# esq4/nind-denoise

Hardware: AMD Instinct MI355X
Metric: megapixels/sec denoised, UtNet cs=256 on 24 MP frames, 1/2/4/8 MI355X (higher is better)
Workload: dtype f32; 1 GPU; configs[1]: one 6000x4000 (24.0 MP) fp32 frame per step, f32 storage in the conv stack (fp32 accumulate), UtNet(funit=64,PReLU) random-init (seed 123), cs=264 (nearest valid to the named size; the reference rejects 256 / 512) ucs=200 ol=64 -> 1276 tiles/frame, tiles per conv-stack launch 256, crop->infer->stitch device resident (frame and canvas in HBM); every tile's input is the whole cs x cs cro; tiles_per_frame=1276, parallelism=single GPU

## Files before the change

nind_denoise_amd/csrc/aux_kernels.hip:

```cpp
#include "nd_common.h"

typedef float f32x4 __attribute__((ext_vector_type(4)));
typedef __bf16 bf16x8 __attribute__((ext_vector_type(8)));
typedef _Float16 f16x8 __attribute__((ext_vector_type(8)));

template <int DT> struct Elem { typedef f32x4 vec; static constexpr int N = 4; typedef float scalar; };
template <> struct Elem<ND_BF16> { typedef bf16x8 vec; static constexpr int N = 8; typedef __bf16 scalar; };
template <> struct Elem<ND_F16> { typedef f16x8 vec; static constexpr int N = 8; typedef _Float16 scalar; };
#define ND_DISPATCH_DT(dt, CALL)                     \
    switch (dt) {                                    \
        case ND_F32: { constexpr int DT = ND_F32; CALL; break; }   \
        case ND_BF16: { constexpr int DT = ND_BF16; CALL; break; } \
        case ND_F16: { constexpr int DT = ND_F16; CALL; break; }   \
        default: ND_FAIL(ND_EINVAL, "unsupported storage type %d", dt); \
    }

static int make_geo(int W, int H, int cs, int ucs, int ol, TileGeo *g) {
    if (W <= 0 || H <= 0 || cs <= 0 || ucs <= 0 || ol < 0) ND_FAIL(ND_EINVAL, "tile grid: non-positive size");
    if (ucs - ol <= 0) ND_FAIL(ND_EINVAL, "tile grid: ucs (%d) must exceed the overlap (%d)", ucs, ol);
    if (cs < ucs) ND_FAIL(ND_EINVAL, "tile grid: cs (%d) < ucs (%d)", cs, ucs);
    g->W = W; g->H = H; g->cs = cs; g->ucs = ucs; g->ol = ol;
    g->stride = ucs - ol;
    g->pad = (cs - ucs) / 2;
    g->cols = ceil_div_py(W - ucs, g->stride) + 1;
// ... 166 lines not shown

int nd_launch_gather_edges(const float *img, int W, int H, int cs, int ucs, int ol, int set, int first, int count, const QpBuf &dst,
                           hipStream_t s) {
    TileGeo g;
    ND_TRY(make_geo(W, H, cs, ucs, ol, &g));
    const bool corners = set == ND_EDGE_CORNERS;
    bool ok = img && dst.base && dst.dt == ND_F32 && dst.pad == 0 && dst.Hb >= 1 && dst.Wb >= 1 && dst.used() <= dst.pstride &&
              dst.B <= 65535 && dst.Hb <= 65535 && first >= 0 && count > 0 && cs >= 3;
    if (set == ND_EDGE_ROWS) ok = ok && first + count <= g.rows && dst.B == 2 * count && dst.Hb <= cs + 4;
    else if (set == ND_EDGE_COLS) ok = ok && first + count <= g.rows && dst.B == 2 * g.cols && dst.Wb <= cs + 4;
    else ok = ok && corners && first + count <= g.cols * g.rows && dst.B == 4 * count && dst.Hb <= cs + 4 && dst.Wb <= cs + 4;
    if (!ok) ND_FAIL(ND_EINVAL, "gather_edges: bad set %d, range [%d,+%d) or destination", set, first, count);
    dim3 grid((dst.Wb + 255) / 256, dst.Hb, dst.B);
    hipLaunchKernelGGL(k_gather_edges, grid, dim3(256), 0, s, img, g, set, first, (f32x4 *)dst.base, dst.Hb, dst.Wb);
    ND_HIP(hipGetLastError());
    return ND_OK;
}

struct SpliceArgs {
    const f32x4 *src;
    f32x4 *dst;
    long src_np, dst_np;
    int src_Hb, src_Wb, src_pad, dst_Hb, dst_Wb, dst_pad;
    int tile_begin, cols, row0, r0, c0, rows, ccols, planes, dst_img0;
    SpliceMap m;
    int band_rows;
    long slot_elems;
};
__global__ void k_splice(SpliceArgs a) {
    const int k = blockIdx.x * blockDim.x + threadIdx.x;
    if (k >= a.rows * a.ccols) return;
    const int r = a.r0 + k / a.ccols, c = a.c0 + k % a.ccols;
    const int t = blockIdx.y / a.planes, p = blockIdx.y - t * a.planes;
    const int i = a.tile_begin + t;
    const int yi = i / a.cols, xi = i - yi * a.cols;
    const int band = a.band_rows > 0 ? yi / a.band_rows : 0, yrel = yi - (a.band_rows > 0 ? band * a.band_rows : a.row0);
    const int simg = a.m.img_t * t + a.m.img_y * yrel + a.m.img_x * xi + a.m.img_add;
    const int sy = yrel * a.m.step_y + r + a.m.oy + a.src_pad, sx = xi * a.m.step_x + c + a.m.ox + a.src_pad;
    const long si = (long)p * a.src_np + (band & 1) * a.slot_elems + ((long)simg * a.src_Hb + sy) * a.src_Wb + sx;
    a.dst[(long)p * a.dst_np + ((long)(a.dst_img0 + t) * a.dst_Hb + r + a.dst_pad) * a.dst_Wb + c + a.dst_pad] = a.src[si];
}

int nd_launch_splice(const QpBuf &src, int src_p0, const QpBuf &dst, int dst_p0, int planes, int tile_begin, int tile_count, int cols,
                     int row0, const SpliceMap &m, int r0, int r1, int c0, int c1, hipStream_t s, int band_rows, long slot_elems,
                     int dst_img0) {
    const int sH = src.Hb - 2 * src.pad, sW = src.Wb - 2 * src.pad, dH = dst.Hb - 2 * dst.pad, dW = dst.Wb - 2 * dst.pad;
    bool ok = src.dt == ND_F32 && dst.dt == ND_F32 && tile_begin >= 0 && cols > 0 && tile_count > 0 && dst_img0 >= 0 &&
              dst_img0 + tile_count <= dst.B && dst.used() <= dst.np() && src.used() <= src.np() && planes > 0 &&
              src_p0 >= 0 && src_p0 + planes <= src.planes && dst_p0 >= 0 && dst_p0 + planes <= dst.planes &&
              r0 >= 0 && c0 >= 0 && r1 > r0 && c1 > c0 && r1 <= dH && c1 <= dW && band_rows >= 0 &&
              (band_rows == 0 || slot_elems >= 0) && (long)tile_count * planes <= 65535;
    for (int t = 0; t < tile_count && ok; ++t) {
        const int yi = (tile_begin + t) / cols, xi = (tile_begin + t) % cols;
        const int yrel = yi - (band_rows > 0 ? yi / band_rows * band_rows : row0);
        const int simg = m.img_t * t + m.img_y * yrel + m.img_x * xi + m.img_add, y = yrel * m.step_y + m.oy, x = xi * m.step_x + m.ox;
        if (band_rows > 0 && (yi / band_rows & 1)) ok = slot_elems >= src.used() && slot_elems + src.used() <= src.np();
        ok = ok && yrel >= 0 && simg >= 0 && simg < src.B && y + r0 >= 0 && y + r1 - 1 < sH && x + c0 >= 0 && x + c1 - 1 < sW;
    }
    if (!ok) ND_FAIL(ND_EINVAL, "splice: region [%d,%d) x [%d,%d) of %d tiles x %d planes outside its source / destination", r0, r1, c0, c1,
                     tile_count, planes);
    SpliceArgs a;
    a.src = (const f32x4 *)src.base + (long)src_p0 * src.np();
    a.dst = (f32x4 *)dst.base + (long)dst_p0 * dst.np();
    a.src_np = src.np(); a.dst_np = dst.np();
    a.src_Hb = src.Hb; a.src_Wb = src.Wb; a.src_pad = src.pad;
    a.dst_Hb = dst.Hb; a.dst_Wb = dst.Wb; a.dst_pad = dst.pad;
    a.tile_begin = tile_begin; a.cols = cols; a.row0 = row0; a.m = m; a.dst_img0 = dst_img0;
    a.r0 = r0; a.c0 = c0; a.rows = r1 - r0; a.ccols = c1 - c0; a.planes = planes;
    a.band_rows = band_rows; a.slot_elems = slot_elems;
    dim3 grid(((r1 - r0) * (c1 - c0) + 255) / 256, tile_count * planes);
    hipLaunchKernelGGL(k_splice, grid, dim3(256), 0, s, a);
    ND_HIP(hipGetLastError());
    return ND_OK;
}

__host__ __device__ static inline long skip_origin(int i, int cols, int band_rows, int step, int Wb, int dpad, long slot_elems) {
    const int yi = i / cols, xi = i - yi * cols, band = yi / band_rows;
    return (band & 1) * slot_elems + (long)((yi - band * band_rows) * step + dpad) * Wb + xi * step + dpad;
}
__global__ void k_skip_origins(int tile_begin, int tile_count, int cols, int band_rows, int step, int Wb, int dpad, long slot_elems,
                               int *__restrict__ table) {
    const int t = blockIdx.x * blockDim.x + threadIdx.x;
    if (t >= tile_count) return;
    table[t] = (int)skip_origin(tile_begin + t, cols, band_rows, step, Wb, dpad, slot_elems);
}

int nd_launch_skip_origins(const QpBuf &src, int dst_pad, int tile_begin, int tile_count, int cols, int band_rows, int step, long slot_elems,
                           int *table, long *origin_max, hipStream_t s) {
    const int dpad = src.pad - dst_pad;
    if (!table || tile_begin < 0 || tile_count <= 0 || cols <= 0 || band_rows <= 0 || step < 0 || dpad < 0 || slot_elems < 0 || src.B != 1)
        ND_FAIL(ND_EINVAL, "skip_origins: bad tile range [%d,+%d) / %d rows per band", tile_begin, tile_count, band_rows);
    long omax = 0;
    for (int t = 0; t < tile_count; ++t) {
        const long o = skip_origin(tile_begin + t, cols, band_rows, step, src.Wb, dpad, slot_elems);
        omax = o > omax ? o : omax;
    }
// ... 499 lines not shown
```

nind_denoise_amd/csrc/conv_w2d.hip:

```cpp
#include "conv_qp.inc"

namespace {

typedef float f32x2 __attribute__((ext_vector_type(2)));

constexpr int kR = 8;
constexpr int kS = 16;
constexpr int kRI = kR + 2;
constexpr int kVPlane = kRI * kS * 16;
constexpr int kVPos = 2 * kVPlane;
constexpr int kVBytes = 6 * kVPos;
constexpr int kTaps = 18;
constexpr int kMTB = 2;
constexpr int kWBytes = kMTB * kTaps * 1024;
constexpr int kStage = kWBytes + kVBytes;
constexpr int kStages = 2;
constexpr int kScratch = 2048;
constexpr int kLds = kStages * kStage + 8 * kScratch;
constexpr int kDmaAt = 4;
constexpr int kXfAt = 12;
constexpr int kSlots = 4 * 32 * 4;

template <int OFF> __device__ __forceinline__ void glds16o(const void *g, void *l) {
    __builtin_amdgcn_global_load_lds((const __attribute__((address_space(1))) void *)g, (__attribute__((address_space(3))) void *)l, 16, OFF, 0);
// ... 6 lines not shown
    v[0] = 4.f * d[0] - 5.f * d[2] + d[4];
    v[1] = s34 - 4.f * s12;
    v[2] = d43 + 4.f * d12;
    v[3] = d42 + 2.f * d31;
    v[4] = d42 - 2.f * d31;
    v[5] = 4.f * d[1] - 5.f * d[3] + d[5];
}
__device__ __forceinline__ void w4_out(const float *m, float *y) {
    const float a = m[1] + m[2], b = m[1] - m[2], c = m[3] + m[4], e = m[3] - m[4];
    y[0] = m[0] + a + c;
    y[1] = b + 2.f * e;
    y[2] = a + 4.f * c;
    y[3] = b + 8.f * e + m[5];
}

__device__ __forceinline__ unsigned long long stamp() {
    unsigned long long t;
    __builtin_amdgcn_sched_barrier(0);
    asm volatile("s_memtime %0\n\ts_waitcnt lgkmcnt(0)" : "=s"(t)::"memory");
    __builtin_amdgcn_sched_barrier(0);
    return t;
}

struct Strip { int img, y0, x0; bool ok; };

template <int DBG, bool SRC2 = false, bool ADD = false>
__global__ __launch_bounds__(512) void conv_w2d(ConvParams p) {
    extern __shared__ __attribute__((aligned(16))) char smem[];
    const int lane = threadIdx.x & 63;
    const int wave = __builtin_amdgcn_readfirstlane(threadIdx.x >> 6);
    const int wm = wave >> 2, wn = wave & 3;
    const int j = lane & 31, h = lane >> 5;
    const int nwg = gridDim.x;
    const int bid = blockIdx.x;
    const int vb = (nwg % 8 == 0) ? (bid % 8) * (nwg / 8) + bid / 8 : bid;

    const int nchunks = p.KB;
    const int nitems = p.nitems;
    const int my_items = vb < nitems ? (nitems - vb + nwg - 1) / nwg : 0;
    struct Item { int tile, c0, c1, slice; };
    auto decode = [&](int w) -> Item {
        Item it;
        if (w < p.split_first) {
            it.tile = w; it.c0 = 0; it.c1 = nchunks; it.slice = -1;
        } else {
            const int u = w - p.split_first;
// ... 465 lines not shown
    const int Hfull = d.in.Hb - 2, Wfull = d.in.Wb - 2;
    if (Hfull < 1 || Wfull < 1) ND_FAIL(ND_EINVAL, "w2d: input smaller than the kernel");
    ND_TRY(nd_check_roi("w2d", d, Hfull, Wfull, d.pool != nullptr, "a pooled layer"));
    const bool roi = d.roi_rows > 0;
    const int Hv = roi ? d.roi_rows : Hfull, Wpx = roi ? d.roi_cols : Wfull, Wg = (Wpx + 3) / 4, NB = (Hv + kR - 1) / kR;
    if (d.pre && (roi || d.pool)) ND_FAIL(ND_EINVAL, "w2d: a pre-activation copy goes with whole, unpooled layers only");
    if (d.cout % 4) ND_FAIL(ND_EINVAL, "w2d: cout must be a multiple of 4");
    ND_TRY(nd_check_in_planes("w2d", d, KB, true, true));
    const bool src2 = d.in2.base != nullptr, add = d.add.base != nullptr;
    if (add && (d.pool || d.pre || src2))
        ND_FAIL(ND_EINVAL, "w2d: a layer with an addend source is neither pooled nor keeps a pre-activation copy nor has a second input source");
    if (add) ND_TRY(nd_check_add("w2d", d, (long)(d.roi_r0 + Hv - 1 + d.add.pad) * d.add.Wb + d.roi_c0 + Wpx - 1 + d.add.pad + 1));
    if (src2 && (d.pool || d.pre)) ND_FAIL(ND_EINVAL, "w2d: a layer with a second input source is neither pooled nor keeps a pre-activation copy");
    if (src2) ND_TRY(nd_check_in2("w2d", d, KB, (long)(d.roi_r0 + (NB - 1) * kR + kRI - 1) * d.in2.Wb + d.roi_c0 + 4 * (Wg - 1) + 6));
    ND_TRY(nd_check_out("w2d", d, Hfull, Wfull, false));
    ND_TRY(nd_check_int32("w2d", d.in));
    if (2 * d.in.np() * 16 + 65536 >= (1L << 32)) ND_FAIL(ND_EINVAL, "w2d: input too large for 32-bit byte offsets");

    int dev = 0, ncus = 0;
    ND_TRY(nd_device(&dev, &ncus));
    void (*fn)(ConvParams) = add ? conv_w2d<0, false, true> : src2 ? conv_w2d<0, true> : conv_w2d<0>;
#ifdef ND_QP_STAMPS
    static const int dbg_all = getenv("ND_W2D_DBG") ? atoi(getenv("ND_W2D_DBG")) : 0;
    const int dbg_env = src2 || add ? 0 : dbg_all;
    switch (dbg_env) {
        case 1: fn = conv_w2d<1>; break;
        case 2: fn = conv_w2d<2>; break;
        case 4: fn = conv_w2d<4>; break;
        case 8: fn = conv_w2d<8>; break;
        case 16: fn = conv_w2d<16>; break;
        case 24: fn = conv_w2d<24>; break;
        case 28: fn = conv_w2d<28>; break;
        case 30: fn = conv_w2d<30>; break;
        case 32: fn = conv_w2d<32>; break;
        case 62: fn = conv_w2d<62>; break;
        case 128: fn = conv_w2d<128>; break;
        case 256: fn = conv_w2d<256>; break;
        default: break;
    }
#endif
    ND_TRY(nd_raise_lds(dev, (const void *)fn, kLds));

    ConvParams p = nd_conv_params(d, KB, d.cout);
    if (roi) {
        p.in += (long)d.roi_r0 * d.in.Wb + d.roi_c0;
        p.out += (long)d.roi_r0 * d.out.Wb + d.roi_c0;
    }
    if (src2) {
        p.in2 = (const f32x4 *)d.in2.base + (long)d.in2_plane0 * d.in2.np() + (roi ? (long)d.roi_r0 * d.in2.Wb + d.roi_c0 : 0);
        p.in2_plane = d.in2.np();
        p.origin2 = d.in2_origin;
        p.kb2 = d.in2_from / 2;
        p.Wb2 = d.in2.Wb;
    }
    if (d.w_kb) {
        p.KBw = d.w_kb;
        p.wpk += (size_t)d.w_kb0 * kTaps * 256;
    }
    if (add) {
        p.add = (const f32x4 *)d.add.base + (long)d.add_plane0 * d.add.np() + (long)((roi ? d.roi_r0 : 0) + d.add.pad) * d.add.Wb +
                (roi ? d.roi_c0 : 0) + d.add.pad;
        p.add_plane = d.add.np();
        p.origin_add = d.add_origin;
        p.W_add = d.add.Wb;
    }
    p.Hv = Hv;
    p.Wv = Wg;
    p.PV = NB * Wg;
    p.wpx = Wpx;
    if (d.pool) {
        ND_TRY(nd_conv_pool("w2d", d, Hv, Wpx, p));
        if (d.pool->used() * 16 >= (1L << 32)) ND_FAIL(ND_EINVAL, "w2d: pooled destination too large for 32-bit byte offsets");
    }
    nd_conv_tiles(p, true, kS, kMTB * 32);
    nd_conv_fastdivs(p);
    const long ntiles = p.tiles_per_problem;
    const long cap = d.part && !d.nosplit && !d.pool && !d.pre ? (long)(d.part_bytes / ((size_t)kMTB * 32 * kSlots * 4)) : 0;
    const long grid = nd_conv_schedule(p, ntiles, KB, ncus, cap);
    p.part = (f32x4 *)d.part;
#ifdef ND_QP_STAMPS
    if (dbg_env == 128) {
        static int printed = 0;
        static const char *const names[6] = {"issue loads + DMA", "MFMA loop", "wait vmcnt", "transform+publish (inside the loop)", "epilogue", "barrier"};
        return nd_stamped_launch(fn, 512, kLds, p, ntiles, KB, ncus, stream, printed++ < 2, nullptr, "[w2d stamps] wave", names, 6, {0, 1, 4});
    }
#endif
    hipLaunchKernelGGL(fn, dim3((unsigned)grid), dim3(512), kLds, stream, p);
    if (p.split_first < ntiles) hipLaunchKernelGGL(k_w2d_split_finish, dim3((unsigned)(ntiles - p.split_first), kMTB * 8), dim3(256), 0, stream, p);
    ND_HIP(hipGetLastError());
    return ND_OK;
}

bool nd_f43_w2d(const QpBuf &in, int cout, bool pre, int flags) {
    return !(flags & ND_FLAG_W1D_REGS) && nd_w2d_ok(in) && (!pre || nd_w2d_tiles(in, cout) >= 512);
}
int nd_launch_conv_f43(const ConvDesc &d, int flags, hipStream_t stream) {
    return nd_f43_w2d(d.in, d.cout, d.pre != nullptr, flags) ? nd_launch_conv_w2d(d, stream) : nd_launch_conv_w1d(4, d, stream);
}
```

nind_denoise_amd/csrc/nd_common.h:

```cpp
#pragma once
#include <hip/hip_runtime.h>

#include <stdarg.h>
#include <stdint.h>
#include <stdio.h>

#include "nind_hip.h"

void nd_set_error(const char *fmt, ...);
#define ND_FAIL(code, ...)        \
    do {                          \
        nd_set_error(__VA_ARGS__); \
        return (code);            \
    } while (0)
#define ND_HIP(call)                                                                         \
    do {                                                                                     \
        hipError_t e_ = (call);                                                              \
        if (e_ != hipSuccess) ND_FAIL(ND_EHIP, "%s failed: %s", #call, hipGetErrorString(e_)); \
    } while (0)
#define ND_TRY(call)        \
    do {                    \
        int r_ = (call);    \
        if (r_ != 0) return r_; \
    } while (0)
// ... 167 lines not shown
int nd_launch_qp_to_nchw(const QpBuf &src, int plane0, float *y, int C, hipStream_t s);
int nd_launch_reflect_pack(const float *x_nchw, int B, int H, int W, const QpBuf &dst, hipStream_t s);
int nd_launch_maxpool2(const QpBuf &src, int src_plane0, int planes, const QpBuf &dst, hipStream_t s);
int nd_launch_final1x1(const QpBuf &src, int cin, const float *w, const float *bias, int crop, float *y_nchw, int H,
                       int W, hipStream_t s, int sigmoid = 0);
int nd_launch_final1x1_stitch(const QpBuf &src, int cin, const float *w, const float *bias, int crop, float *canvas,
                              int width, int height, int cs, int ucs, int ol, int tile_begin, int tile_count,
                              hipStream_t s, int sigmoid = 0, const float *noise_img = nullptr);
int nd_launch_gather_pack(const float *img, int width, int height, int cs, int ucs, int ol, int tile_begin,
                          int tile_count, const QpBuf &dst, hipStream_t s, int border = 2, bool reflect = true);
int nd_launch_gather_band(const float *img, int width, int height, int cs, int ucs, int ol, int band_row0, const QpBuf &dst,
                          hipStream_t s);
enum nd_edge_set { ND_EDGE_ROWS = 0, ND_EDGE_COLS = 1, ND_EDGE_CORNERS = 2 };
int nd_launch_gather_edges(const float *img, int width, int height, int cs, int ucs, int ol, int set, int first, int count,
                           const QpBuf &dst, hipStream_t s);
int nd_launch_skip_origins(const QpBuf &src, int dst_pad, int tile_begin, int tile_count, int cols, int band_rows, int step, long slot_elems,
                           int *table, long *origin_max, hipStream_t s);
struct SpliceMap {
    int step_y = 0, step_x = 0, img_t = 0, img_y = 0, img_x = 0, img_add = 0, oy = 0, ox = 0;
};
int nd_launch_splice(const QpBuf &src, int src_p0, const QpBuf &dst, int dst_p0, int planes, int tile_begin, int tile_count, int cols,
                     int row0, const SpliceMap &m, int r0, int r1, int c0, int c1, hipStream_t s, int band_rows = 0,
                     long slot_elems = 0, int dst_img0 = 0);

int nd_launch_repitch(const QpBuf &src, int src_plane0, int planes, int ss, int sy, int sx, const QpBuf &dst, int oy, int ox, int h, int w,
                      hipStream_t s);
size_t nd_wgrad_partial_floats(int taps, int M, int N, long K, int *ksplit_out, int *cps_out);
int nd_launch_wgrad(const QpBuf &A, int a_plane0, int M, const QpBuf &Bq, int b_plane0, int N, int taps, int taps_total, int tap0,
                    float *partial, size_t partial_floats, float *dw, hipStream_t s);
int nd_launch_channel_sum(const QpBuf &src, int plane0, int C, float *out, float *scratch, hipStream_t s);
int nd_launch_maxpool_bwd_add(const QpBuf &gpool, const QpBuf &fwd, int fwd_plane0, const QpBuf &gfine, int g_plane0, int planes,
                              hipStream_t s);
int nd_launch_final_wgrad(const float *gy, int H, int W, const QpBuf &act, int cin, int crop, float *red, float *dw, float *db,
                          hipStream_t s);
int nd_launch_final_bwd_data(const float *gy, int H, int W, const float *w, int cin, int crop, const QpBuf &g, hipStream_t s);

int nd_launch_bn_train_fwd(const QpBuf &z, const QpBuf &a, int plane0, int cout, float momentum, const float *gamma, const float *beta,
                           float *rm, float *rv, float *stat, float *red, long red_floats, hipStream_t s);
int nd_launch_bn_train_bwd(const QpBuf &g, const QpBuf &a, int plane0, const QpBuf &z, int cout, const float *gamma, const float *stat,
                           float *coef, float *dgamma, float *dbeta, float *red, long red_floats, hipStream_t s);
```

nind_denoise_amd/csrc/utnet_frame.hip:

```cpp
#include <string.h>

#include "nd_common.h"

#include "utnet_net.h"

namespace {

constexpr int kSharedSteps = 6, kLevel2End = 9;
constexpr int kStrip = 16, kStrip2 = 6;
constexpr double kBandBytes = 8.0 * (1 << 30);

struct Level {
    int begin, end;
    Buf in, out;
    int strip;
    int out_shift;
    bool three_pass;
    bool by_side;
};
const Level kLevels[2] = {{0, kSharedSteps, X0, P2, kStrip, 2, false, false}, {kSharedSteps, kLevel2End, P2, P3, kStrip2, 3, true, true}};
struct SkipSpec { Buf cat; int level, edge; };
const SkipSpec kSkips[3] = {{CAT4, 0, 2}, {CAT3, 0, 1}, {CAT2, 1, 1}};
inline int skip_step(Buf cat) {
    for (int i = 0; i < kNumSteps; ++i)
// ... 252 lines not shown
    struct Skip { int step; bool in_place, fold; Form form; } skips[3];
    int skip_planes(int k) const { return pl.buf[kSkips[k].cat].planes / 2; }
    int tile_rows(int b) const { return fp.rows - b * fp.R < fp.R ? fp.rows - b * fp.R : fp.R; }
};

inline Plan level_scratch(const Frame &c, int l, Plan p) {
    p.split = c.pl.split;
    p.wino = c.ws.scratch[l];
    p.wino_bytes = c.fp.lb[l].scratch;
    return p;
}
inline int run_level(const Frame &c, int l, const Plan &p) {
    StackOpts o;
    o.flags = c.flags;
    o.step_begin = kLevels[l].begin;
    o.step_end = kLevels[l].end;
    return run_stack(c.f, c.act, c.dt, c.blob, p, c.s, o);
}
inline void line_image(const Level &lv, int side, int count, int *step, int *add) {
    *step = lv.by_side ? 1 : 2;
    *add = lv.by_side ? side * count : side;
}

int splice_line_inputs(const Frame &c, int l, int nrows, const Plan &band, const Plan &re, const Plan &ce, const Plan &rows, const Plan &cols) {
    const Level &lv = kLevels[l], &up = kLevels[l - 1];
    const Buf in = lv.in;
    const int n = c.tile[in], planes = band.buf[in].planes, h = band.buf[in].Hb, w = band.buf[in].Wb;
    for (int side = 0; side < 2; ++side) {
        const int at = side * (lv.strip - 1), in0 = 1 - side, in1 = lv.strip - side;
        SpliceMap br, lr, bc, lc;
        br.step_y = bc.step_x = c.fp.S >> up.out_shift;
        br.oy = bc.ox = side * (n - lv.strip);
        line_image(up, side, nrows, &lr.img_y, &lr.img_add);
        line_image(up, side, c.fp.cols, &lc.img_x, &lc.img_add);
        lr.oy = lc.ox = -at;
        ND_TRY(nd_launch_splice(band.buf[in], 0, rows.buf[in], 0, planes, 0, nrows, 1, 0, br, in0, in1, 0, w, c.s, 0, 0, side * nrows));
        ND_TRY(nd_launch_splice(re.buf[in], 0, rows.buf[in], 0, planes, 0, nrows, 1, 0, lr, at, at + 1, 0, w, c.s, 0, 0, side * nrows));
        ND_TRY(nd_launch_splice(band.buf[in], 0, cols.buf[in], 0, planes, 0, c.fp.cols, c.fp.cols, 0, bc, 0, h, in0, in1, c.s, 0, 0, side * c.fp.cols));
        ND_TRY(nd_launch_splice(ce.buf[in], 0, cols.buf[in], 0, planes, 0, c.fp.cols, c.fp.cols, 0, lc, 0, h, at, at + 1, c.s, 0, 0, side * c.fp.cols));
    }
    return ND_OK;
}

int build_band(const Frame &c, int b) {
    const FramePlan &fp = c.fp;
    const int row0 = b * fp.R, nrows = c.tile_rows(b), slot = b & 1;
    Plan band, re, ce;
    for (int l = 0; l < c.nlev; ++l) {
        const Level &lv = kLevels[l];
        Plan bp = level_scratch(c, l, band_plan(fp, l, c.f, c.dt, nrows, c.cs, c.ws.band[l], slot));
        if (l == 0)
            ND_TRY(nd_launch_gather_band(c.img, c.W, c.H, c.cs, c.ucs, c.ol, row0, bp.buf[lv.in], c.s));
        else
            bp.buf[lv.in] = band.buf[lv.in];
        ND_TRY(run_level(c, l, bp));
        for (int k = 0; k < 3; ++k)
            if (kSkips[k].level == l && c.skips[k].fold)
                ND_TRY(launch_skip_fold(c.f, c.flags, c.blob, c.bl, c.skips[k].step, c.skips[k].form, bp.buf[kSkips[k].cat], c.skip_planes(k),
                                        c.rois[c.skips[k].step], fp.S >> k, nrows, fp.cols, c.pl.split, c.ws.fold_scratch, fp.fold_bytes, c.s));
        const Plan rows = level_scratch(c, l, row_plan(fp, l, c.f, c.dt, nrows, c.ws.rows[l], slot));
        const Plan cols = level_scratch(c, l, col_plan(fp, l, c.f, c.dt, nrows, c.cs, c.ws.cols[l], slot));
        if (l == 0) {
            ND_TRY(nd_launch_gather_edges(c.img, c.W, c.H, c.cs, c.ucs, c.ol, ND_EDGE_ROWS, row0, nrows, rows.buf[lv.in], c.s));
            ND_TRY(nd_launch_gather_edges(c.img, c.W, c.H, c.cs, c.ucs, c.ol, ND_EDGE_COLS, row0, nrows, cols.buf[lv.in], c.s));
        } else {
            ND_TRY(splice_line_inputs(c, l, nrows, band, re, ce, rows, cols));
        }
        ND_TRY(run_level(c, l, rows));
        ND_TRY(run_level(c, l, cols));
        band = bp;
        re = rows;
        ce = cols;
    }
    return ND_OK;
}

int corner_patches(const Frame &c, int l, const Plan &tp, int t0, int cnt, Plan *cp) {
    const Level &lv = kLevels[l];
    *cp = level_scratch(c, l, corner_plan(l, c.f, c.dt, cnt, c.batch, c.ws.corners[l]));
    if (l == 0) ND_TRY(nd_launch_gather_edges(c.img, c.W, c.H, c.cs, c.ucs, c.ol, ND_EDGE_CORNERS, t0, cnt, cp->buf[lv.in], c.s));
    for (int k = 0; l > 0 && k < 4; ++k) {
        SpliceMap m;
        m.img_t = 1;
        m.oy = (k >> 1) * (c.tile[lv.in] - lv.strip);
        m.ox = (k & 1) * (c.tile[lv.in] - lv.strip);
        ND_TRY(nd_launch_splice(tp.buf[lv.in], 0, cp->buf[lv.in], 0, tp.buf[lv.in].planes, 0, cnt, cnt, 0, m, 0, lv.strip, 0, lv.strip, c.s, 0, 0, k * cnt));
    }
    return run_level(c, l, *cp);
}

int bind_skips(const Frame &c, const Plan &tp, int t0, int cnt, StepSrc2 *src2, int *nsrc2) {
    const FramePlan &fp = c.fp;
    *nsrc2 = 0;
    for (int k = 0; k < 3; ++k) {
        if (kSkips[k].level >= c.nlev) continue;
        const Buf cat = kSkips[k].cat;
        const QpBuf &src = c.full[kSkips[k].level].buf[cat];
        const int planes = c.skip_planes(k), tstep = fp.S >> k, *win = fp.win[k];
        if (!c.skips[k].in_place && !c.skips[k].fold) {
            SpliceMap m;
            m.step_y = m.step_x = tstep;
            ND_TRY(nd_launch_splice(src, planes, tp.buf[cat], planes, planes, t0, cnt, fp.cols, 0, m, win[0], win[1], win[0], win[1], c.s, fp.R,
                                    slot_elems(src, fp.slots)));
            continue;
        }
        StepSrc2 &q = src2[(*nsrc2)++];
        q.step = c.skips[k].step;
        q.buf = src;
        q.plane0 = q.from = planes;
        q.addend = c.skips[k].fold;
        if (q.addend) {
            q.plane0 = 0;
            q.buf.pad = 1;
        }
        q.origin = c.ws.origins[k];
        ND_TRY(nd_launch_skip_origins(src, tp.buf[cat].pad, t0, cnt, fp.cols, fp.R, tstep, slot_elems(src, fp.slots), c.ws.origins[k],
                                      &q.origin_max, c.s));
    }
    return ND_OK;
}

int assemble_output(const Frame &c, int l, const Plan &tp, const Plan &cp, int t0, int cnt) {
    const FramePlan &fp = c.fp;
    const Level &lv = kLevels[l];
    const QpBuf &dst = tp.buf[lv.out], &bt = c.full[l].buf[lv.out];
    const int n = c.tile[lv.out], step = fp.S >> lv.out_shift, per_band = fp.R * fp.cols;
    SpliceMap whole;
    whole.step_y = whole.step_x = step;
    ND_TRY(nd_launch_splice(bt, 0, dst, 0, dst.planes, t0, cnt, fp.cols, 0, whole, 0, n, 0, n, c.s, fp.R, slot_elems(bt, fp.slots)));
    for (int b = t0 / per_band; b <= (t0 + cnt - 1) / per_band; ++b) {
        const int lo = t0 > b * per_band ? t0 : b * per_band, hi = t0 + cnt < (b + 1) * per_band ? t0 + cnt : (b + 1) * per_band;
        const int row0 = b * fp.R, nrows = c.tile_rows(b);
        const QpBuf rl = row_plan(fp, l, c.f, c.dt, nrows, c.ws.rows[l], b & 1).buf[lv.out];
        const QpBuf cl = col_plan(fp, l, c.f, c.dt, nrows, c.cs, c.ws.cols[l], b & 1).buf[lv.out];
        for (int side = 0; side < 2; ++side) {
            const int at = side * (n - 1);
            SpliceMap mr, mc;
            mr.step_x = mc.step_y = step;
            line_image(lv, side, nrows, &mr.img_y, &mr.img_add);
            line_image(lv, side, fp.cols, &mc.img_x, &mc.img_add);
            mr.oy = mc.ox = -at;
            ND_TRY(nd_launch_splice(rl, 0, dst, 0, dst.planes, lo, hi - lo, fp.cols, row0, mr, at, at + 1, 0, n, c.s, 0, 0, lo - t0));
            ND_TRY(nd_launch_splice(cl, 0, dst, 0, dst.planes, lo, hi - lo, fp.cols, row0, mc, 0, n, at, at + 1, c.s, 0, 0, lo - t0));
        }
    }
    for (int k = 0; k < 4; ++k) {
        const int r = (k >> 1) * (n - 1), col = (k & 1) * (n - 1);
        SpliceMap m;
        m.img_t = lv.by_side ? 1 : 4;
        m.img_add = lv.by_side ? k * cnt : k;
        m.oy = -r;
        m.ox = -col;
        ND_TRY(nd_launch_splice(cp.buf[lv.out], 0, dst, 0, dst.planes, t0, cnt, fp.cols, 0, m, r, r + 1, col, col + 1, c.s));
    }
    return ND_OK;
}

}

extern "C" size_t nd_utnet_frame_workspace_bytes(int funit, int dtype, int flags, int width, int height, int cs, int ucs, int ol,
                                                 int batch) {
    FramePlan fp;
    if (nd_check_flags(flags, true) != ND_OK || frame_plan(funit, dtype, flags, width, height, cs, ucs, ol, batch, &fp) != ND_OK) return 0;
    return fp.bytes;
}

extern "C" int nd_utnet_frame_plan(int funit, int dtype, int flags, int width, int height, int cs, int ucs, int ol, int *out) {
    ND_TRY(nd_check_flags(flags, true));
    if (!out) ND_FAIL(ND_EINVAL, "nd_utnet_frame_plan: null output");
    FramePlan fp;
    ND_TRY(frame_plan(funit, dtype, flags, width, height, cs, ucs, ol, 1, &fp));
    const int v[8] = {fp.D, fp.aligned, fp.R, fp.nbands, fp.S, fp.cols, fp.rows, fp.in_h[0]};
    memcpy(out, v, sizeof(v));
    return ND_OK;
}

extern "C" int nd_utnet_frame_levels(int funit, int dtype, int flags, int width, int height, int cs, int ucs, int ol, int *levels) {
    ND_TRY(nd_check_flags(flags, true));
// ... 87 lines not shown
```

nind_denoise_amd/csrc/winograd.hip:

```cpp
#include <stdlib.h>

#include <algorithm>
#include <atomic>
#include <thread>
#include <vector>

#include "nd_common.h"

typedef float f32x4 __attribute__((ext_vector_type(4)));

namespace {

__device__ __forceinline__ void tile_pos(long t, int TX, int TY, int &tx, int &ty, int &b) {
    const unsigned u = (unsigned)t, row = u / (unsigned)TX;
    tx = (int)(u - row * (unsigned)TX);
    b = (int)(row / (unsigned)TY);
    ty = (int)(row - (unsigned)b * (unsigned)TY);
}

template <int T> struct Wino;
template <> struct Wino<2> {
    static constexpr int A = 4;
    template <typename V> __host__ __device__ static void bt(const V *d, V *o) {
        o[0] = d[0] - d[2];
// ... 264 lines not shown
                                                             const int *__restrict__ origin_add = nullptr, int W_add = 0, int mp = 0,
                                                             int mbx = 0, int mby = 0) {
    static_assert(!(MOSAIC && ADD), "the mosaic form has no addend");
    constexpr int A = Wino<T>::A, RS = T * A + 1, NTH = NTL * A;
    __shared__ f32x4 sr[NTL * RS];
    __shared__ f32x4 so[T][NTL * T];
    const long tiles = MOSAIC ? (long)TY * TX : (long)B * TY * TX;
    const long t0 = (long)blockIdx.x * NTL;
    const int q = blockIdx.y;
    const f32x4 bv = ADD ? f32x4{0.f, 0.f, 0.f, 0.f} : *(const f32x4 *)(bias + 4 * q);
    const float slope = act == ND_ACT_NONE ? 1.f : (slope_dev ? *slope_dev : slope_imm);
    auto activate = [&](f32x4 y) {
#pragma unroll
        for (int e = 0; e < 4; ++e) {
            const float u = y[e];
            switch (act) {
                case ND_ACT_ELU: y[e] = u > 0.f ? u : expm1f(u); break;
                case ND_ACT_HARDSWISH: y[e] = u * fminf(fmaxf(u + 3.f, 0.f), 6.f) / 6.f; break;
                default: y[e] = u > 0.f ? u : u * slope; break;
            }
        }
        return y;
    };
    {
        const int j = threadIdx.x / NTL, tl = threadIdx.x % NTL;
        const long t = t0 + tl;
        if (t < tiles) {
            const f32x4 *src = m + (long)q * mnp + t;
            f32x4 c[A], o[T];
#pragma unroll
            for (int i = 0; i < A; ++i) c[i] = src[(long)(i * A + j) * mbs];
            Wino<T>::at(c, o);
#pragma unroll
            for (int i = 0; i < T; ++i) sr[tl * RS + i * A + j] = o[i];
        }
    }
    __syncthreads();
    if (threadIdx.x < NTL * T) {
        const int i = threadIdx.x / NTL, tl = threadIdx.x % NTL;
        if (t0 + tl < tiles) {
            f32x4 r[A], o[T];
#pragma unroll
            for (int j = 0; j < A; ++j) r[j] = sr[tl * RS + i * A + j];
            Wino<T>::at(r, o);
#pragma unroll
            for (int j = 0; j < T; ++j) {
                so[i][tl * T + j] = ADD ? o[j] : activate(o[j] + bv);
            }
        }
    }
    __syncthreads();
    f32x4 *dst = out + (long)(out_plane0 + q) * onp;
    for (int idx = threadIdx.x; idx < T * NTL * T; idx += NTH) {
        const int i = idx / (NTL * T), pp = idx - i * (NTL * T);
        const long tt = t0 + pp / T;
        if (tt >= tiles) continue;
        int tx, ty, b;
        tile_pos(tt, TX, TY, tx, ty, b);
        const int xx = T * tx + pp % T, yy = T * ty + i;
        if constexpr (MOSAIC) {
            const unsigned cx = (unsigned)xx / (unsigned)mp, cy = (unsigned)yy / (unsigned)mp;
            const int lx = xx - (int)cx * mp, ly = yy - (int)cy * mp, bi = (int)cy * mbx + (int)cx;
            if ((int)cx < mbx && (int)cy < mby && bi < B) dst[(long)bi * out_img_stride + (long)(ly + opad) * Wo + lx + opad] = so[i][pp];
        } else if (xx < Wv && yy < Hv) {
            f32x4 y = so[i][pp];
            if constexpr (ADD) y = activate(y + add[(long)q * add_np + (long)origin_add[b] + (long)yy * W_add + xx]);
            dst[(long)b * out_img_stride + (long)(yy + opad) * Wo + xx + opad] = y;
        }
    }
    if (!ADD && !MOSAIC && pool) {
        f32x4 *pd = pool + (long)q * pnp;
        for (int idx = threadIdx.x; idx < (T / 2) * NTL * (T / 2); idx += NTH) {
            const int a = idx / (NTL * (T / 2)), pp = idx - a * (NTL * (T / 2));
            const int tl = pp / (T / 2), c = pp % (T / 2);
            const long tt = t0 + tl;
            if (tt >= tiles) continue;
            int tx, ty, b;
        tile_pos(tt, TX, TY, tx, ty, b);
            const int px = tx * (T / 2) + c, py = ty * (T / 2) + a;
            if (2 * px + 1 < Wv && 2 * py + 1 < Hv) {
                const f32x4 p00 = so[2 * a][tl * T + 2 * c], p01 = so[2 * a][tl * T + 2 * c + 1];
                const f32x4 p10 = so[2 * a + 1][tl * T + 2 * c], p11 = so[2 * a + 1][tl * T + 2 * c + 1];
                f32x4 v;
#pragma unroll
                for (int e = 0; e < 4; ++e) v[e] = fmaxf(fmaxf(p00[e], p01[e]), fmaxf(p10[e], p11[e]));
                pd[((long)b * Hp + py + ppad) * Wp + px + ppad] = v;
            }
        }
    }
}
// ... 268 lines not shown
```

Before: 89.61 MP/s.

## Batch splice launches into multi-job kernel and prefetch addend in Winograd epilogue

Adds a multi-job splice kernel that takes up to 16 splice regions in one launch, and routes the line, corner and tile-assembly splices through a job list. The goal is fewer small kernel launches per level. The whole-tile splice is also trimmed to its interior or to the four strip corners, so border rows and columns covered by other jobs are not copied twice. The Winograd ADD epilogue now loads the addend values before the transform and barriers, hiding their latency. Debug stamp options are extended as well, at the cost of more host-side validation and a larger kernel argument block.

```diff
diff --git a/nind_denoise_amd/csrc/aux_kernels.hip b/nind_denoise_amd/csrc/aux_kernels.hip
--- a/nind_denoise_amd/csrc/aux_kernels.hip
+++ b/nind_denoise_amd/csrc/aux_kernels.hip
@@ -212,16 +212,26 @@
     f32x4 *dst;
     long src_np, dst_np;
     int src_Hb, src_Wb, src_pad, dst_Hb, dst_Wb, dst_pad;
-    int tile_begin, cols, row0, r0, c0, rows, ccols, planes, dst_img0;
+    int tile_begin, tiles, cols, row0, r0, c0, rows, ccols, planes, dst_img0;
     SpliceMap m;
     int band_rows;
     long slot_elems;
 };
-__global__ void k_splice(SpliceArgs a) {
-    const int k = blockIdx.x * blockDim.x + threadIdx.x;
-    if (k >= a.rows * a.ccols) return;
+struct SpliceJobArgs {
+    SpliceArgs job[kSpliceJobs];
+    int first[kSpliceJobs + 1];
+    int n;
+};
+__global__ __launch_bounds__(256) void k_splice_jobs(SpliceJobArgs ja) {
+    int j = 0;
+    while (j + 1 < ja.n && (int)blockIdx.x >= ja.first[j + 1]) ++j;
+    const SpliceArgs &a = ja.job[j];
+    const int npix = a.rows * a.ccols;
+    const int e = ((int)blockIdx.x - ja.first[j]) * 256 + (int)threadIdx.x;
+    const int y = e / npix, k = e - y * npix;
+    const int t = y / a.planes, p = y - t * a.planes;
+    if (t >= a.tiles) return;
     const int r = a.r0 + k / a.ccols, c = a.c0 + k % a.ccols;
-    const int t = blockIdx.y / a.planes, p = blockIdx.y - t * a.planes;
     const int i = a.tile_begin + t;
     const int yi = i / a.cols, xi = i - yi * a.cols;
     const int band = a.band_rows > 0 ? yi / a.band_rows : 0, yrel = yi - (a.band_rows > 0 ? band * a.band_rows : a.row0);
@@ -231,37 +241,72 @@
     a.dst[(long)p * a.dst_np + ((long)(a.dst_img0 + t) * a.dst_Hb + r + a.dst_pad) * a.dst_Wb + c + a.dst_pad] = a.src[si];
 }
 
+static bool splice_jobs_overlap(const SpliceJob &a, const SpliceJob &b) {
+    auto meet = [](long a0, long a1, long b0, long b1) { return a0 < b1 && b0 < a1; };
+    const QpBuf &p = a.dst, &q = b.dst;
+    if (p.base == q.base && p.Hb == q.Hb && p.Wb == q.Wb && p.pad == q.pad && p.np() == q.np())
+        return meet(a.dst_p0, a.dst_p0 + a.planes, b.dst_p0, b.dst_p0 + b.planes) &&
+               meet(a.dst_img0, a.dst_img0 + a.tile_count, b.dst_img0, b.dst_img0 + b.tile_count) && meet(a.r0, a.r1, b.r0, b.r1) &&
+               meet(a.c0, a.c1, b.c0, b.c1);
+    const uintptr_t pa = (uintptr_t)p.base, pb = (uintptr_t)q.base;
+    return meet(pa + (size_t)a.dst_p0 * p.np() * 16, pa + (size_t)(a.dst_p0 + a.planes) * p.np() * 16, pb + (size_t)b.dst_p0 * q.np() * 16,
+                pb + (size_t)(b.dst_p0 + b.planes) * q.np() * 16);
+}
+
+int nd_launch_splices(const SpliceJob *jobs, int n, hipStream_t s) {
+    if (!jobs || n < 1 || n > kSpliceJobs) ND_FAIL(ND_EINVAL, "splice: %d jobs in one launch (1 ... %d)", n, kSpliceJobs);
+    SpliceJobArgs ja;
+    long blocks = 0;
+    for (int j = 0; j < n; ++j) {
+        const SpliceJob &q = jobs[j];
+        const QpBuf &src = q.src, &dst = q.dst;
+        const int sH = src.Hb - 2 * src.pad, sW = src.Wb - 2 * src.pad, dH = dst.Hb - 2 * dst.pad, dW = dst.Wb - 2 * dst.pad;
+        bool ok = src.base && dst.base && src.dt == ND_F32 && dst.dt == ND_F32 && q.tile_begin >= 0 && q.cols > 0 && q.tile_count > 0 &&
+                  q.dst_img0 >= 0 && q.dst_img0 + q.tile_count <= dst.B && dst.used() <= dst.np() && src.used() <= src.np() && q.planes > 0 &&
+                  q.src_p0 >= 0 && q.src_p0 + q.planes <= src.planes && q.dst_p0 >= 0 && q.dst_p0 + q.planes <= dst.planes &&
+                  q.r0 >= 0 && q.c0 >= 0 && q.r1 > q.r0 && q.c1 > q.c0 && q.r1 <= dH && q.c1 <= dW && q.band_rows >= 0 &&
+                  (q.band_rows == 0 || q.slot_elems >= 0);
+        const long elems = ok ? (long)q.tile_count * q.planes * (q.r1 - q.r0) * (q.c1 - q.c0) : 0;
+        ok = ok && elems <= 0x7fffffffL - 256;
+        for (int t = 0; t < q.tile_count && ok; ++t) {
+            const int yi = (q.tile_begin + t) / q.cols, xi = (q.tile_begin + t) % q.cols;
+            const int yrel = yi - (q.band_rows > 0 ? yi / q.band_rows * q.band_rows : q.row0);
+            const int simg = q.m.img_t * t + q.m.img_y * yrel + q.m.img_x * xi + q.m.img_add, y = yrel * q.m.step_y + q.m.oy,
+                      x = xi * q.m.step_x + q.m.ox;
+            if (q.band_rows > 0 && (yi / q.band_rows & 1)) ok = q.slot_elems >= src.used() && q.slot_elems + src.used() <= src.np();
+            ok = ok && yrel >= 0 && simg >= 0 && simg < src.B && y + q.r0 >= 0 && y + q.r1 - 1 < sH && x + q.c0 >= 0 && x + q.c1 - 1 < sW;
+        }
+        if (!ok) ND_FAIL(ND_EINVAL, "splice: job %d, region [%d,%d) x [%d,%d) of %d tiles x %d planes outside its source / destination", j,
+                         q.r0, q.r1, q.c0, q.c1, q.tile_count, q.planes);
+        for (int i = 0; i < j; ++i)
+            if (splice_jobs_overlap(jobs[i], q)) ND_FAIL(ND_EINVAL, "splice: jobs %d and %d write overlapping regions", i, j);
+        SpliceArgs &a = ja.job[j];
+        a.src = (const f32x4 *)src.base + (long)q.src_p0 * src.np();
+        a.dst = (f32x4 *)dst.base + (long)q.dst_p0 * dst.np();
+        a.src_np = src.np(); a.dst_np = dst.np();
+        a.src_Hb = src.Hb; a.src_Wb = src.Wb; a.src_pad = src.pad;
+        a.dst_Hb = dst.Hb; a.dst_Wb = dst.Wb; a.dst_pad = dst.pad;
+        a.tile_begin = q.tile_begin; a.tiles = q.tile_count; a.cols = q.cols; a.row0 = q.row0; a.m = q.m; a.dst_img0 = q.dst_img0;
+        a.r0 = q.r0; a.c0 = q.c0; a.rows = q.r1 - q.r0; a.ccols = q.c1 - q.c0; a.planes = q.planes;
+        a.band_rows = q.band_rows; a.slot_elems = q.slot_elems;
+        ja.first[j] = (int)blocks;
+        blocks += (elems + 255) / 256;
+        if (blocks * 256 >= (1L << 32)) ND_FAIL(ND_EINVAL, "splice: %ld blocks of 256 threads in one launch", blocks);
+    }
+    for (int j = n; j < kSpliceJobs; ++j) ja.job[j] = ja.job[0];
+    for (int j = n; j <= kSpliceJobs; ++j) ja.first[j] = (int)blocks;
+    ja.n = n;
+    hipLaunchKernelGGL(k_splice_jobs, dim3((unsigned)blocks), dim3(256), 0, s, ja);
+    ND_HIP(hipGetLastError());
+    return ND_OK;
+}
+
 int nd_launch_splice(const QpBuf &src, int src_p0, const QpBuf &dst, int dst_p0, int planes, int tile_begin, int tile_count, int cols,
                      int row0, const SpliceMap &m, int r0, int r1, int c0, int c1, hipStream_t s, int band_rows, long slot_elems,
                      int dst_img0) {
-    const int sH = src.Hb - 2 * src.pad, sW = src.Wb - 2 * src.pad, dH = dst.Hb - 2 * dst.pad, dW = dst.Wb - 2 * dst.pad;
-    bool ok = src.dt == ND_F32 && dst.dt == ND_F32 && tile_begin >= 0 && cols > 0 && tile_count > 0 && dst_img0 >= 0 &&
-              dst_img0 + tile_count <= dst.B && dst.used() <= dst.np() && src.used() <= src.np() && planes > 0 &&
-              src_p0 >= 0 && src_p0 + planes <= src.planes && dst_p0 >= 0 && dst_p0 + planes <= dst.planes &&
-              r0 >= 0 && c0 >= 0 && r1 > r0 && c1 > c0 && r1 <= dH && c1 <= dW && band_rows >= 0 &&
-              (band_rows == 0 || slot_elems >= 0) && (long)tile_count * planes <= 65535;
-    for (int t = 0; t < tile_count && ok; ++t) {
-        const int yi = (tile_begin + t) / cols, xi = (tile_begin + t) % cols;
-        const int yrel = yi - (band_rows > 0 ? yi / band_rows * band_rows : row0);
-        const int simg = m.img_t * t + m.img_y * yrel + m.img_x * xi + m.img_add, y = yrel * m.step_y + m.oy, x = xi * m.step_x + m.ox;
-        if (band_rows > 0 && (yi / band_rows & 1)) ok = slot_elems >= src.used() && slot_elems + src.used() <= src.np();
-        ok = ok && yrel >= 0 && simg >= 0 && simg < src.B && y + r0 >= 0 && y + r1 - 1 < sH && x + c0 >= 0 && x + c1 - 1 < sW;
-    }
-    if (!ok) ND_FAIL(ND_EINVAL, "splice: region [%d,%d) x [%d,%d) of %d tiles x %d planes outside its source / destination", r0, r1, c0, c1,
-                     tile_count, planes);
-    SpliceArgs a;
-    a.src = (const f32x4 *)src.base + (long)src_p0 * src.np();
-    a.dst = (f32x4 *)dst.base + (long)dst_p0 * dst.np();
-    a.src_np = src.np(); a.dst_np = dst.np();
-    a.src_Hb = src.Hb; a.src_Wb = src.Wb; a.src_pad = src.pad;
-    a.dst_Hb = dst.Hb; a.dst_Wb = dst.Wb; a.dst_pad = dst.pad;
-    a.tile_begin = tile_begin; a.cols = cols; a.row0 = row0; a.m = m; a.dst_img0 = dst_img0;
-    a.r0 = r0; a.c0 = c0; a.rows = r1 - r0; a.ccols = c1 - c0; a.planes = planes;
-    a.band_rows = band_rows; a.slot_elems = slot_elems;
-    dim3 grid(((r1 - r0) * (c1 - c0) + 255) / 256, tile_count * planes);
-    hipLaunchKernelGGL(k_splice, grid, dim3(256), 0, s, a);
-    ND_HIP(hipGetLastError());
-    return ND_OK;
+    const SpliceJob q = nd_splice_job(src, src_p0, dst, dst_p0, planes, tile_begin, tile_count, cols, row0, m, r0, r1, c0, c1, band_rows,
+                                      slot_elems, dst_img0);
+    return nd_launch_splices(&q, 1, s);
 }
 
 __host__ __device__ static inline long skip_origin(int i, int cols, int band_rows, int step, int Wb, int dpad, long slot_elems) {
diff --git a/nind_denoise_amd/csrc/conv_w2d.hip b/nind_denoise_amd/csrc/conv_w2d.hip
--- a/nind_denoise_amd/csrc/conv_w2d.hip
+++ b/nind_denoise_amd/csrc/conv_w2d.hip
@@ -52,6 +52,9 @@
     return t;
 }
 
+#ifdef ND_QP_STAMPS
+const char *const kStampNames[6] = {"issue loads + DMA", "MFMA loop", "wait vmcnt", "transform+publish (inside the loop)", "epilogue", "barrier"};
+#endif
 struct Strip { int img, y0, x0; bool ok; };
 
 template <int DBG, bool SRC2 = false, bool ADD = false>
@@ -563,7 +566,7 @@
     void (*fn)(ConvParams) = add ? conv_w2d<0, false, true> : src2 ? conv_w2d<0, true> : conv_w2d<0>;
 #ifdef ND_QP_STAMPS
     static const int dbg_all = getenv("ND_W2D_DBG") ? atoi(getenv("ND_W2D_DBG")) : 0;
-    const int dbg_env = src2 || add ? 0 : dbg_all;
+    const int dbg_env = src2 ? 0 : add ? (dbg_all == 128 ? 128 : 0) : dbg_all;
     switch (dbg_env) {
         case 1: fn = conv_w2d<1>; break;
         case 2: fn = conv_w2d<2>; break;
@@ -575,7 +578,7 @@
         case 30: fn = conv_w2d<30>; break;
         case 32: fn = conv_w2d<32>; break;
         case 62: fn = conv_w2d<62>; break;
-        case 128: fn = conv_w2d<128>; break;
+        case 128: fn = add ? conv_w2d<128, false, true> : conv_w2d<128>; break;
         case 256: fn = conv_w2d<256>; break;
         default: break;
     }
@@ -621,9 +624,15 @@
     p.part = (f32x4 *)d.part;
 #ifdef ND_QP_STAMPS
     if (dbg_env == 128) {
-        static int printed = 0;
-        static const char *const names[6] = {"issue loads + DMA", "MFMA loop", "wait vmcnt", "transform+publish (inside the loop)", "epilogue", "barrier"};
-        return nd_stamped_launch(fn, 512, kLds, p, ntiles, KB, ncus, stream, printed++ < 2, nullptr, "[w2d stamps] wave", names, 6, {0, 1, 4});
+        static const int only_kb = getenv("ND_W2D_STAMP_KB") ? atoi(getenv("ND_W2D_STAMP_KB")) : 0;
+        static int printed = 0, printed_kb[2] = {0, 0};
+        char header[160];
+        snprintf(header, sizeof(header), "[w2d stamps] kind %d cin %d cout %d KB %d tiles %ld%s", d.kind, d.cin, d.cout, KB, ntiles,
+                 add ? " ADDEND" : "");
+        if (only_kb)
+            return nd_stamped_launch(fn, 512, kLds, p, ntiles, KB, ncus, stream, KB == only_kb && ntiles >= 4 * ncus && printed_kb[add]++ < 4,
+                                     header, "[w2d stamps] wave", kStampNames, 6, {0, 1, 4});
+        return nd_stamped_launch(fn, 512, kLds, p, ntiles, KB, ncus, stream, printed++ < 2, nullptr, "[w2d stamps] wave", kStampNames, 6, {0, 1, 4});
     }
 #endif
     hipLaunchKernelGGL(fn, dim3((unsigned)grid), dim3(512), kLds, stream, p);
diff --git a/nind_denoise_amd/csrc/nd_common.h b/nind_denoise_amd/csrc/nd_common.h
--- a/nind_denoise_amd/csrc/nd_common.h
+++ b/nind_denoise_amd/csrc/nd_common.h
@@ -213,6 +213,21 @@
 int nd_launch_splice(const QpBuf &src, int src_p0, const QpBuf &dst, int dst_p0, int planes, int tile_begin, int tile_count, int cols,
                      int row0, const SpliceMap &m, int r0, int r1, int c0, int c1, hipStream_t s, int band_rows = 0,
                      long slot_elems = 0, int dst_img0 = 0);
+struct SpliceJob {
+    QpBuf src, dst;
+    int src_p0, dst_p0, planes, tile_begin, tile_count, cols, row0;
+    SpliceMap m;
+    int r0, r1, c0, c1, band_rows;
+    long slot_elems;
+    int dst_img0;
+};
+constexpr int kSpliceJobs = 16;
+static inline SpliceJob nd_splice_job(const QpBuf &src, int src_p0, const QpBuf &dst, int dst_p0, int planes, int tile_begin, int tile_count,
+                                      int cols, int row0, const SpliceMap &m, int r0, int r1, int c0, int c1, int band_rows = 0,
+                                      long slot_elems = 0, int dst_img0 = 0) {
+    return SpliceJob{src, dst, src_p0, dst_p0, planes, tile_begin, tile_count, cols, row0, m, r0, r1, c0, c1, band_rows, slot_elems, dst_img0};
+}
+int nd_launch_splices(const SpliceJob *jobs, int n, hipStream_t s);
 
 int nd_launch_repitch(const QpBuf &src, int src_plane0, int planes, int ss, int sy, int sx, const QpBuf &dst, int oy, int ox, int h, int w,
                       hipStream_t s);
diff --git a/nind_denoise_amd/csrc/utnet_frame.hip b/nind_denoise_amd/csrc/utnet_frame.hip
--- a/nind_denoise_amd/csrc/utnet_frame.hip
+++ b/nind_denoise_amd/csrc/utnet_frame.hip
@@ -298,10 +298,27 @@
     *add = lv.by_side ? side * count : side;
 }
 
+struct SpliceList {
+    hipStream_t s;
+    SpliceJob job[kSpliceJobs];
+    int n = 0;
+    int flush() {
+        const int k = n;
+        n = 0;
+        return k ? nd_launch_splices(job, k, s) : ND_OK;
+    }
+    int add(const SpliceJob &j) {
+        if (n == kSpliceJobs) ND_TRY(flush());
+        job[n++] = j;
+        return ND_OK;
+    }
+};
+
 int splice_line_inputs(const Frame &c, int l, int nrows, const Plan &band, const Plan &re, const Plan &ce, const Plan &rows, const Plan &cols) {
     const Level &lv = kLevels[l], &up = kLevels[l - 1];
     const Buf in = lv.in;
     const int n = c.tile[in], planes = band.buf[in].planes, h = band.buf[in].Hb, w = band.buf[in].Wb;
+    SpliceList jobs = {c.s};
     for (int side = 0; side < 2; ++side) {
         const int at = side * (lv.strip - 1), in0 = 1 - side, in1 = lv.strip - side;
         SpliceMap br, lr, bc, lc;
@@ -310,12 +327,12 @@
         line_image(up, side, nrows, &lr.img_y, &lr.img_add);
         line_image(up, side, c.fp.cols, &lc.img_x, &lc.img_add);
         lr.oy = lc.ox = -at;
-        ND_TRY(nd_launch_splice(band.buf[in], 0, rows.buf[in], 0, planes, 0, nrows, 1, 0, br, in0, in1, 0, w, c.s, 0, 0, side * nrows));
-        ND_TRY(nd_launch_splice(re.buf[in], 0, rows.buf[in], 0, planes, 0, nrows, 1, 0, lr, at, at + 1, 0, w, c.s, 0, 0, side * nrows));
-        ND_TRY(nd_launch_splice(band.buf[in], 0, cols.buf[in], 0, planes, 0, c.fp.cols, c.fp.cols, 0, bc, 0, h, in0, in1, c.s, 0, 0, side * c.fp.cols));
-        ND_TRY(nd_launch_splice(ce.buf[in], 0, cols.buf[in], 0, planes, 0, c.fp.cols, c.fp.cols, 0, lc, 0, h, at, at + 1, c.s, 0, 0, side * c.fp.cols));
-    }
-    return ND_OK;
+        ND_TRY(jobs.add(nd_splice_job(band.buf[in], 0, rows.buf[in], 0, planes, 0, nrows, 1, 0, br, in0, in1, 0, w, 0, 0, side * nrows)));
+        ND_TRY(jobs.add(nd_splice_job(re.buf[in], 0, rows.buf[in], 0, planes, 0, nrows, 1, 0, lr, at, at + 1, 0, w, 0, 0, side * nrows)));
+        ND_TRY(jobs.add(nd_splice_job(band.buf[in], 0, cols.buf[in], 0, planes, 0, c.fp.cols, c.fp.cols, 0, bc, 0, h, in0, in1, 0, 0, side * c.fp.cols)));
+        ND_TRY(jobs.add(nd_splice_job(ce.buf[in], 0, cols.buf[in], 0, planes, 0, c.fp.cols, c.fp.cols, 0, lc, 0, h, at, at + 1, 0, 0, side * c.fp.cols)));
+    }
+    return jobs.flush();
 }
 
 int build_band(const Frame &c, int b) {
@@ -355,13 +372,15 @@
     const Level &lv = kLevels[l];
     *cp = level_scratch(c, l, corner_plan(l, c.f, c.dt, cnt, c.batch, c.ws.corners[l]));
     if (l == 0) ND_TRY(nd_launch_gather_edges(c.img, c.W, c.H, c.cs, c.ucs, c.ol, ND_EDGE_CORNERS, t0, cnt, cp->buf[lv.in], c.s));
+    SpliceList jobs = {c.s};
     for (int k = 0; l > 0 && k < 4; ++k) {
         SpliceMap m;
         m.img_t = 1;
         m.oy = (k >> 1) * (c.tile[lv.in] - lv.strip);
         m.ox = (k & 1) * (c.tile[lv.in] - lv.strip);
-        ND_TRY(nd_launch_splice(tp.buf[lv.in], 0, cp->buf[lv.in], 0, tp.buf[lv.in].planes, 0, cnt, cnt, 0, m, 0, lv.strip, 0, lv.strip, c.s, 0, 0, k * cnt));
-    }
+        ND_TRY(jobs.add(nd_splice_job(tp.buf[lv.in], 0, cp->buf[lv.in], 0, tp.buf[lv.in].planes, 0, cnt, cnt, 0, m, 0, lv.strip, 0, lv.strip, 0, 0, k * cnt)));
+    }
+    ND_TRY(jobs.flush());
     return run_level(c, l, *cp);
 }
 
@@ -401,9 +420,19 @@
     const Level &lv = kLevels[l];
     const QpBuf &dst = tp.buf[lv.out], &bt = c.full[l].buf[lv.out];
     const int n = c.tile[lv.out], step = fp.S >> lv.out_shift, per_band = fp.R * fp.cols;
+    SpliceList jobs = {c.s};
     SpliceMap whole;
     whole.step_y = whole.step_x = step;
-    ND_TRY(nd_launch_splice(bt, 0, dst, 0, dst.planes, t0, cnt, fp.cols, 0, whole, 0, n, 0, n, c.s, fp.R, slot_elems(bt, fp.slots)));
+    const int strip = l + 1 < c.nlev ? kLevels[l + 1].strip : 0;
+    if (strip > 0 && n >= 2 * strip) {
+        for (int k = 0; k < 4; ++k) {
+            const int r0 = (k >> 1) ? n - strip : 1, c0 = (k & 1) ? n - strip : 1;
+            ND_TRY(jobs.add(nd_splice_job(bt, 0, dst, 0, dst.planes, t0, cnt, fp.cols, 0, whole, r0, r0 + strip - 1, c0, c0 + strip - 1, fp.R,
+                                          slot_elems(bt, fp.slots))));
+        }
+    } else {
+        ND_TRY(jobs.add(nd_splice_job(bt, 0, dst, 0, dst.planes, t0, cnt, fp.cols, 0, whole, 1, n - 1, 1, n - 1, fp.R, slot_elems(bt, fp.slots))));
+    }
     for (int b = t0 / per_band; b <= (t0 + cnt - 1) / per_band; ++b) {
         const int lo = t0 > b * per_band ? t0 : b * per_band, hi = t0 + cnt < (b + 1) * per_band ? t0 + cnt : (b + 1) * per_band;
         const int row0 = b * fp.R, nrows = c.tile_rows(b);
@@ -416,8 +445,8 @@
             line_image(lv, side, nrows, &mr.img_y, &mr.img_add);
             line_image(lv, side, fp.cols, &mc.img_x, &mc.img_add);
             mr.oy = mc.ox = -at;
-            ND_TRY(nd_launch_splice(rl, 0, dst, 0, dst.planes, lo, hi - lo, fp.cols, row0, mr, at, at + 1, 0, n, c.s, 0, 0, lo - t0));
-            ND_TRY(nd_launch_splice(cl, 0, dst, 0, dst.planes, lo, hi - lo, fp.cols, row0, mc, 0, n, at, at + 1, c.s, 0, 0, lo - t0));
+            ND_TRY(jobs.add(nd_splice_job(rl, 0, dst, 0, dst.planes, lo, hi - lo, fp.cols, row0, mr, at, at + 1, 1, n - 1, 0, 0, lo - t0)));
+            ND_TRY(jobs.add(nd_splice_job(cl, 0, dst, 0, dst.planes, lo, hi - lo, fp.cols, row0, mc, 1, n - 1, at, at + 1, 0, 0, lo - t0)));
         }
     }
     for (int k = 0; k < 4; ++k) {
@@ -427,9 +456,9 @@
         m.img_add = lv.by_side ? k * cnt : k;
         m.oy = -r;
         m.ox = -col;
-        ND_TRY(nd_launch_splice(cp.buf[lv.out], 0, dst, 0, dst.planes, t0, cnt, fp.cols, 0, m, r, r + 1, col, col + 1, c.s));
-    }
-    return ND_OK;
+        ND_TRY(jobs.add(nd_splice_job(cp.buf[lv.out], 0, dst, 0, dst.planes, t0, cnt, fp.cols, 0, m, r, r + 1, col, col + 1)));
+    }
+    return jobs.flush();
 }
 
 }
diff --git a/nind_denoise_amd/csrc/winograd.hip b/nind_denoise_amd/csrc/winograd.hip
--- a/nind_denoise_amd/csrc/winograd.hip
+++ b/nind_denoise_amd/csrc/winograd.hip
@@ -310,6 +310,28 @@
         }
         return y;
     };
+    auto pixel_of = [&](int idx, int &i, int &pp, int &b, int &yy, int &xx) {
+        i = idx / (NTL * T);
+        pp = idx - i * (NTL * T);
+        const long tt = t0 + pp / T;
+        if (idx >= T * NTL * T || tt >= tiles) return false;
+        int tx, ty;
+        tile_pos(tt, TX, TY, tx, ty, b);
+        xx = T * tx + pp % T;
+        yy = T * ty + i;
+        return xx < Wv && yy < Hv;
+    };
+    constexpr int NADD = ADD ? (T * NTL * T + NTH - 1) / NTH : 1;
+    f32x4 av[NADD];
+    if constexpr (ADD) {
+        const f32x4 *ap = add + (long)q * add_np;
+#pragma unroll
+        for (int it = 0; it < NADD; ++it) {
+            int i, pp, b, yy, xx;
+            const bool ok = pixel_of(threadIdx.x + it * NTH, i, pp, b, yy, xx);
+            av[it] = ap[ok ? (long)origin_add[b] + (long)yy * W_add + xx : 0L];
+        }
+    }
     {
         const int j = threadIdx.x / NTL, tl = threadIdx.x % NTL;
         const long t = t0 + tl;
@@ -339,21 +361,29 @@
     }
     __syncthreads();
     f32x4 *dst = out + (long)(out_plane0 + q) * onp;
-    for (int idx = threadIdx.x; idx < T * NTL * T; idx += NTH) {
-        const int i = idx / (NTL * T), pp = idx - i * (NTL * T);
-        const long tt = t0 + pp / T;
-        if (tt >= tiles) continue;
-        int tx, ty, b;
-        tile_pos(tt, TX, TY, tx, ty, b);
-        const int xx = T * tx + pp % T, yy = T * ty + i;
-        if constexpr (MOSAIC) {
-            const unsigned cx = (unsigned)xx / (unsigned)mp, cy = (unsigned)yy / (unsigned)mp;
-            const int lx = xx - (int)cx * mp, ly = yy - (int)cy * mp, bi = (int)cy * mbx + (int)cx;
-            if ((int)cx < mbx && (int)cy < mby && bi < B) dst[(long)bi * out_img_stride + (long)(ly + opad) * Wo + lx + opad] = so[i][pp];
-        } else if (xx < Wv && yy < Hv) {
-            f32x4 y = so[i][pp];
-            if constexpr (ADD) y = activate(y + add[(long)q * add_np + (long)origin_add[b] + (long)yy * W_add + xx]);
-            dst[(long)b * out_img_stride + (long)(yy + opad) * Wo + xx + opad] = y;
+    if constexpr (ADD) {
+#pragma unroll
+        for (int it = 0; it < NADD; ++it) {
+            int i, pp, b, yy, xx;
+            if (pixel_of(threadIdx.x + it * NTH, i, pp, b, yy, xx))
+                dst[(long)b * out_img_stride + (long)(yy + opad) * Wo + xx + opad] = activate(so[i][pp] + av[it]);
+        }
+    }
+    if constexpr (!ADD) {
+        for (int idx = threadIdx.x; idx < T * NTL * T; idx += NTH) {
+            const int i = idx / (NTL * T), pp = idx - i * (NTL * T);
+            const long tt = t0 + pp / T;
+            if (tt >= tiles) continue;
+            int tx, ty, b;
+            tile_pos(tt, TX, TY, tx, ty, b);
+            const int xx = T * tx + pp % T, yy = T * ty + i;
+            if constexpr (MOSAIC) {
+                const unsigned cx = (unsigned)xx / (unsigned)mp, cy = (unsigned)yy / (unsigned)mp;
+                const int lx = xx - (int)cx * mp, ly = yy - (int)cy * mp, bi = (int)cy * mbx + (int)cx;
+                if ((int)cx < mbx && (int)cy < mby && bi < B) dst[(long)bi * out_img_stride + (long)(ly + opad) * Wo + lx + opad] = so[i][pp];
+            } else if (xx < Wv && yy < Hv) {
+                dst[(long)b * out_img_stride + (long)(yy + opad) * Wo + xx + opad] = so[i][pp];
+            }
         }
     }
     if (!ADD && !MOSAIC && pool) {
```

Measured after the change: 90.58 MP/s, median of 6. 1.1% higher.
